# HKUDS/SSLRec

Measured on AMD Instinct MI355X. Metric: propagation_edges_per_sec, higher is better.
Workload: dtype f32

## Files before the change

include/sslrec_hip.h:

```cpp
#ifndef SSLREC_HIP_H
#define SSLREC_HIP_H

#include <stddef.h>
#include <stdint.h>

#ifdef __cplusplus
extern "C" {
#endif

#define SSLREC_ABI_VERSION 7
#define SSLREC_E_BADARG 1001

int sslrec_abi_version(void);

int sslrec_row_bits3(const int64_t *idx0, int64_t off0, const int64_t *idx1, int64_t off1, const int64_t *idx2, int64_t off2,
                     int32_t n, int32_t n_rows, uint32_t *bits, void *stream);

typedef struct sslrec_csr {
    int32_t n_rows, n_cols, nnz;
    int32_t d;
    int32_t n_elem;
    const int32_t *col;
    const float   *val;
    int32_t n_waves;
// ... 118 lines not shown
                             int32_t *w_len_out, void *stream);

typedef struct sslrec_plan sslrec_plan_t;
#define SSLREC_PLAN_AUTO 0
#define SSLREC_PLAN_SWEPT 1
#define SSLREC_PLAN_STREAMED 2
#define SSLREC_PLAN_BUNDLED 3
#define SSLREC_PLAN_NO_XCD_SPLIT 1
typedef struct sslrec_plan_info {
    int32_t n_rows, n_cols; int64_t nnz;
    int32_t kind, d, xcd_split;
    int32_t n_elem, n_blocks, n_slots, n_streams, n_rseg, n_long;
    int64_t xcd_col_pairs;
} sslrec_plan_info_t;
int sslrec_plan_build_coo(const int64_t *rows, const int64_t *cols, const float *vals, int64_t nnz, int32_t n_rows,
                          int32_t n_cols, sslrec_plan_t **out);
int sslrec_plan_build_csr(const int64_t *rowptr, const int32_t *col, const float *val, int32_t n_rows, int32_t n_cols,
                          sslrec_plan_t **out);
int sslrec_plan_set_option(sslrec_plan_t *p, const char *name, int64_t value);
int sslrec_plan_layout(sslrec_plan_t *p, int32_t d, int32_t kind, int32_t flags);
int sslrec_plan_info(const sslrec_plan_t *p, int32_t d, int32_t kind, sslrec_plan_info_t *info);
int sslrec_plan_host_array(const sslrec_plan_t *p, int32_t d, int32_t kind, const char *name, const void **ptr, int64_t *count,
                           int32_t *elem_bytes);
int sslrec_plan_upload(sslrec_plan_t *p, int32_t d, int32_t kind, void *stream);
const sslrec_swept_t *sslrec_plan_swept(const sslrec_plan_t *p, int32_t d);
const sslrec_csr_t *sslrec_plan_csr(const sslrec_plan_t *p, int32_t d);
const sslrec_bundled_t *sslrec_plan_bundled(const sslrec_plan_t *p, int32_t d);
const int32_t *sslrec_plan_edge_map(const sslrec_plan_t *p, int32_t d, int32_t kind);
int sslrec_plan_spmm_f32(const sslrec_plan_t *p, int32_t d, const float *X, float *Y, const sslrec_epilogue_t *epi,
                         void *stream);
void sslrec_plan_free(sslrec_plan_t *p);

int sslrec_debug_swept_trace(int enable, unsigned long long *host_out, int n_waves);

int sslrec_debug_stamp_next_launch(unsigned long long *record);
int sslrec_debug_wall_clock_khz(void);

size_t sslrec_bpr_ws_bytes(int32_t B);
size_t sslrec_bpr_bwd_ws_bytes(int32_t B, int32_t d);
int sslrec_bpr_fwd_f32(const float *Ta, const int64_t *ia, const float *Tp, const int64_t *ip,
                       const float *Tn, const int64_t *in, int32_t B, int32_t d, int32_t variant,
                       float divisor, float *ws, float *loss_out, void *stream);
int sslrec_bpr_fwd_total_f32(const float *Ta, const int64_t *ia, const float *Tp, const int64_t *ip,
                             const float *Tn, const int64_t *in, int32_t B, int32_t d, int32_t variant,
                             float divisor, const float *add_in, float *ws, float *loss_out2, void *stream);
int sslrec_bpr_bwd_f32(const float *Ta, const int64_t *ia, const float *Tp, const int64_t *ip,
                       const float *Tn, const int64_t *in, int32_t B, int32_t d, int32_t variant, float divisor,
                       const float *gscale_dev, float *dTa, float *dTp, float *dTn, void *ws, void *stream);
int sslrec_bpr_bwd_table_init(void *ws, int32_t B, int32_t d, void *stream);
int sslrec_bpr_bwd_kept_f32(const float *Ta, const int64_t *ia, const float *Tp, const int64_t *ip,
                            const float *Tn, const int64_t *in, int32_t B, int32_t d, int32_t variant, float divisor,
                            const float *gscale_dev, float *dTa, float *dTp, float *dTn, void *ws, float *zero_table,
                            size_t zero_elems, void *stream);

#define SSLREC_INFONCE_PREC_DEFAULT 0
#define SSLREC_INFONCE_PREC_X6 1
#define SSLREC_INFONCE_PREC_FP32 2
#define SSLREC_INFONCE_PREC_X36 3
#define SSLREC_INFONCE_PREC_X3 4
#define SSLREC_INFONCE_PREC_X63 5
#define SSLREC_INFONCE_PREC_X6A 6
#define SSLREC_INFONCE_PREC_H3 7
#define SSLREC_INFONCE_FWD_W (1 << 16)
size_t sslrec_infonce_ws_bytes(int32_t B, int32_t M, int32_t d);
int sslrec_infonce_fwd_f32(const float *T1, const int64_t *i1, const float *T2, const int64_t *i2,
                           int32_t B, const float *ALL, int32_t M, int32_t d, float temp,
                           int32_t variant, float *ws, float *loss_out, void *stream);
int sslrec_infonce_bwd_f32(const float *T1, const int64_t *i1, const float *T2, const int64_t *i2,
                           int32_t B, const float *ALL, int32_t M, int32_t d, float temp,
                           int32_t variant, float *ws, const float *gscale_dev,
                           float *dE1, float *dE2, float *dALL, void *stream);

int sslrec_infonce_bwd_scatter_f32(const float *T1, const int64_t *i1, const float *T2, const int64_t *i2,
                                   int32_t B, const float *ALL, int32_t M, int32_t d, float temp,
                                   int32_t variant, float *ws, const float *gscale_dev, float *dE,
                                   float *dT1, float *dT2, float *dALL, void *scatter_ws, void *stream);

int sslrec_infonce_shard_rowsum_f32(const float *T1, const int64_t *i1, const float *T2, const int64_t *i2,
                                    int32_t B, const float *ALL, int32_t M, int32_t d, float temp,
                                    int32_t variant, float *ws, float *z_part, void *stream);
int sslrec_infonce_shard_loss_f32(int32_t B, int32_t M, int32_t d, int32_t variant, float *ws,
                                  const float *z_total, float *loss_out, void *stream);
int sslrec_infonce_shard_bwd_f32(int32_t B, int32_t M, int32_t d, float temp, int32_t variant, float *ws,
                                 const float *gscale_dev, float *w_part, float *dALL, void *stream);
int sslrec_infonce_shard_finish_bwd_f32(int32_t B, int32_t M, int32_t d, float temp, int32_t variant,
                                        float *ws, const float *gscale_dev, const float *w_total,
                                        float *dE1, float *dE2, void *stream);

size_t sslrec_sumsq_ws_bytes(void);
int sslrec_sumsq_fwd_f32(const float *x, size_t n, float weight, float *ws, float *out, void *stream);
int sslrec_sumsq_bwd_f32(const float *x, size_t n, float weight, const float *gscale_dev, float *dx, void *stream);

int sslrec_weighted_sum4_f32(const float *t0, float w0, const float *t1, float w1, const float *t2, float w2, const float *t3, float w3,
                             float *out6, void *stream);
int sslrec_scalar_scale2_f32(const float *x, float a, float b, float *out2, void *stream);
int sslrec_add_tables_f32(const float *a, const float *b, const float *c, float *out, size_t n, void *stream);

int sslrec_adam_tick(float *state, double lr, double beta1, double beta2, void *stream);
int sslrec_adam_apply_f32(float *p, const float *g, float *m, float *v, size_t n, const float *state,
                          double beta1, double beta2, double eps, double weight_decay, void *stream);

size_t sslrec_rankq_ws_bytes(int32_t q, int32_t d);
int sslrec_rankq_reduce_f32(const float *M, int64_t stride_q, int64_t stride_n, const float *X, int32_t N, int32_t d,
                            int32_t q, float *ws, float *out, void *stream);
int sslrec_rankq_expand_f32(const float *M, int64_t stride_q, int64_t stride_n, const float *S, int32_t N, int32_t d,
                            int32_t q, float *Y, void *stream);
// ... 27 lines not shown
```

sslrec_amd/_lib.py:

```python
import ctypes as C
import os
import subprocess

_HERE = os.path.dirname(os.path.abspath(__file__))
CSRC = os.path.join(_HERE, 'csrc')
SO_PATH = os.environ.get('SSLREC_HIP_LIBRARY') or os.path.join(CSRC, 'libsslrec_hip.so')

E_BADARG = 1001
EXPECTED_ABI = 7


class CsrStruct(C.Structure):
    _fields_ = [
        ('n_rows', C.c_int32), ('n_cols', C.c_int32), ('nnz', C.c_int32), ('d', C.c_int32), ('n_elem', C.c_int32),
        ('col', C.c_void_p), ('val', C.c_void_p),
        ('n_waves', C.c_int32),
        ('w_start', C.c_void_p), ('w_len', C.c_void_p), ('r_ptr', C.c_void_p),
        ('n_rseg', C.c_int32),
        ('r_len', C.c_void_p), ('r_dst', C.c_void_p),
        ('n_long', C.c_int32),
        ('long_row', C.c_void_p), ('long_ptr', C.c_void_p),
        ('n_slots', C.c_int32),
    ]

# ... 55 lines not shown
    'sslrec_debug_stamp_next_launch': (C.c_int, [C.c_void_p]),
    'sslrec_debug_wall_clock_khz': (C.c_int, []),
    'sslrec_philox_row_sumsq': (C.c_int, [_P, C.c_uint32, _I, _I, _P, _P]),
    'sslrec_row_sumsq_f32': (C.c_int, [_P, _I, _I, _P, _P]),
    'sslrec_debug_gather_rows': (C.c_int, [_P, C.c_uint32, _I, _I, _I, _P, _P, _P]),
    'sslrec_debug_swept_trace': (C.c_int, [C.c_int, _P, C.c_int]),
    'sslrec_spmm_csr_f32': (C.c_int, [C.POINTER(CsrStruct), _P, _P, _P, _P, _P, _I, _P, C.POINTER(EpilogueStruct), _P, _P]),
    'sslrec_spmm_bundled_f32': (C.c_int, [C.POINTER(BundledStruct), _P, _P, _I, _P, C.POINTER(EpilogueStruct), _P, _P]),
    'sslrec_spmm_swept_f32': (C.c_int, [C.POINTER(SweptStruct), _P, _P, _P, _P, _I, _P, C.POINTER(EpilogueStruct), _P]),
    'sslrec_swept_deferred_sum_ok': (C.c_int, [C.POINTER(SweptStruct)]),
    'sslrec_spmm_swept_views_f32': (C.c_int, [C.POINTER(SweptStruct), _P, _I, C.POINTER(EpilogueViewsStruct), _P]),
    'sslrec_swept_compact': (C.c_int, [C.POINTER(SweptStruct), _P, _P, _F, _P, _P, _P, _P]),
    'sslrec_edge_drop_compact': (C.c_int, [C.POINTER(CsrStruct), _P, _P, _F, _P, _P, _P, _P, _P]),
    'sslrec_full_predict_f32': (C.c_int, [_P, _P, _I, _P, _I, _I, _P, _I, _P, _P]),
    'sslrec_eval_topk_ws_bytes': (C.c_size_t, [_I, _I, _I]),
    'sslrec_eval_topk_f32': (C.c_int, [_P, _P, _I, _P, _I, _I, _P, _P, _I, _P, _P, _P, _P]),
    'sslrec_sample_negs': (C.c_int, [_P, C.c_int64, _P, _P, _I, _P, C.c_uint32, _P, _P]),
    'sslrec_sample_negs_mt19937': (C.c_int, [_P, _P, _P, C.c_int64, _P, _P, _I, _I, _P, _P]),
    'sslrec_philox_advance': (C.c_int, [_P, _P]),
    'sslrec_philox_fill_f32': (C.c_int, [_P, C.c_uint32, _P, C.c_size_t, _P]),
    'sslrec_mt19937_uniform_f32': (C.c_int, [_P, _P, C.c_int64, _P]),
    'sslrec_mt19937_keep_mask': (C.c_int, [_P, C.c_float, _P, C.c_int64, _P]),
    'sslrec_mt19937_jump_poly': (C.c_int, [_P, _P, _P, _P]),
    'sslrec_mt19937_par_ws_bytes': (C.c_size_t, [C.c_int32, C.c_int32]),
    'sslrec_mt19937_uniform_par_f32': (C.c_int, [_P, _P, C.c_int32, C.c_int32, C.c_int64, _P, _P, C.c_int64, _P]),
    'sslrec_mt19937_keep_mask_par': (C.c_int, [_P, _P, C.c_int32, C.c_int32, C.c_int64, _P, C.c_float, _P, C.c_int64, _P]),
    'sslrec_swept_compact_philox': (C.c_int, [C.POINTER(SweptStruct), _P, _F, _P, C.c_uint32, _F, _P, _P, _P, _P]),
    'sslrec_edge_drop_compact_philox': (C.c_int, [C.POINTER(CsrStruct), _P, _F, _P, C.c_uint32, _F, _P, _P, _P, _P, _P]),
    'sslrec_bundled_drop_values': (C.c_int, [C.POINTER(BundledStruct), _P, _P, _F, _P, C.c_uint32, _F, _P, _P]),
    'sslrec_bundled_compact': (C.c_int, [C.POINTER(BundledStruct), _P, _P, _F, _P, _P, _P, _P, _P]),
    'sslrec_bundled_compact_philox': (C.c_int, [C.POINTER(BundledStruct), _P, _F, _P, C.c_uint32, _F, _P, _P, _P, _P, _P]),
    'sslrec_spmm_bundled_view_f32': (C.c_int, [C.POINTER(BundledStruct), _P, _P, _P, _P, _P, _I, _P, C.POINTER(EpilogueStruct), _P, _P]),
    'sslrec_plan_build_coo': (C.c_int, [_P, _P, _P, C.c_int64, _I, _I, C.POINTER(C.c_void_p)]),
    'sslrec_plan_build_csr': (C.c_int, [_P, _P, _P, _I, _I, C.POINTER(C.c_void_p)]),
    'sslrec_plan_set_option': (C.c_int, [_P, C.c_char_p, C.c_int64]),
    'sslrec_plan_layout': (C.c_int, [_P, _I, _I, _I]),
    'sslrec_plan_info': (C.c_int, [_P, _I, _I, C.POINTER(PlanInfoStruct)]),
    'sslrec_plan_host_array': (C.c_int, [_P, _I, _I, C.c_char_p, C.POINTER(C.c_void_p), C.POINTER(C.c_int64), C.POINTER(C.c_int32)]),
    'sslrec_plan_upload': (C.c_int, [_P, _I, _I, _P]),
    'sslrec_plan_swept': (C.c_void_p, [_P, _I]),
    'sslrec_plan_csr': (C.c_void_p, [_P, _I]),
    'sslrec_plan_bundled': (C.c_void_p, [_P, _I]),
    'sslrec_plan_edge_map': (C.c_void_p, [_P, _I, _I]),
    'sslrec_plan_spmm_f32': (C.c_int, [_P, _I, _P, _P, C.POINTER(EpilogueStruct), _P]),
    'sslrec_plan_free': (None, [_P]),
    'sslrec_bpr_ws_bytes': (C.c_size_t, [_I]),
    'sslrec_bpr_fwd_f32': (C.c_int, [_P, _P, _P, _P, _P, _P, _I, _I, _I, _F, _P, _P, _P]),
    'sslrec_bpr_fwd_total_f32': (C.c_int, [_P, _P, _P, _P, _P, _P, _I, _I, _I, _F, _P, _P, _P, _P]),
    'sslrec_bpr_bwd_ws_bytes': (C.c_size_t, [_I, _I]),
    'sslrec_scatter_ws_bytes': (C.c_size_t, [_I]),
    'sslrec_bpr_bwd_f32': (C.c_int, [_P, _P, _P, _P, _P, _P, _I, _I, _I, _F, _P, _P, _P, _P, _P, _P]),
    'sslrec_bpr_bwd_table_init': (C.c_int, [_P, _I, _I, _P]),
    'sslrec_bpr_bwd_kept_f32': (C.c_int, [_P, _P, _P, _P, _P, _P, _I, _I, _I, _F, _P, _P, _P, _P, _P, _P, C.c_size_t, _P]),
    'sslrec_infonce_ws_bytes': (C.c_size_t, [_I, _I, _I]),
    'sslrec_infonce_fwd_f32': (C.c_int, [_P, _P, _P, _P, _I, _P, _I, _I, _F, _I, _P, _P, _P]),
    'sslrec_infonce_bwd_f32': (C.c_int, [_P, _P, _P, _P, _I, _P, _I, _I, _F, _I, _P, _P, _P, _P, _P, _P]),
    'sslrec_infonce_bwd_scatter_f32': (C.c_int, [_P, _P, _P, _P, _I, _P, _I, _I, _F, _I, _P, _P, _P, _P, _P, _P, _P, _P]),
    'sslrec_infonce_shard_rowsum_f32': (C.c_int, [_P, _P, _P, _P, _I, _P, _I, _I, _F, _I, _P, _P, _P]),
    'sslrec_infonce_shard_loss_f32': (C.c_int, [_I, _I, _I, _I, _P, _P, _P, _P]),
    'sslrec_infonce_shard_bwd_f32': (C.c_int, [_I, _I, _I, _F, _I, _P, _P, _P, _P, _P]),
    'sslrec_infonce_shard_finish_bwd_f32': (C.c_int, [_I, _I, _I, _F, _I, _P, _P, _P, _P, _P, _P]),
    'sslrec_adam_tick': (C.c_int, [_P, C.c_double, C.c_double, C.c_double, _P]),
    'sslrec_adam_apply_f32': (C.c_int, [_P, _P, _P, _P, C.c_size_t, _P, C.c_double, C.c_double, C.c_double, C.c_double, _P]),
    'sslrec_rankq_ws_bytes': (C.c_size_t, [_I, _I]),
    'sslrec_rankq_reduce_f32': (C.c_int, [_P, C.c_int64, C.c_int64, _P, _I, _I, _I, _P, _P, _P]),
    'sslrec_rankq_expand_f32': (C.c_int, [_P, C.c_int64, C.c_int64, _P, _I, _I, _I, _P, _P]),
    'sslrec_scatter_add_rows_f32': (C.c_int, [_P, _P, _I, _I, _P, _P, _P]),
    'sslrec_sumsq_ws_bytes': (C.c_size_t, []),
    'sslrec_sumsq_fwd_f32': (C.c_int, [_P, C.c_size_t, _F, _P, _P, _P]),
    'sslrec_sumsq_bwd_f32': (C.c_int, [_P, C.c_size_t, _F, _P, _P, _P]),
    'sslrec_weighted_sum4_f32': (C.c_int, [_P, _F, _P, _F, _P, _F, _P, _F, _P, _P]),
    'sslrec_scalar_scale2_f32': (C.c_int, [_P, _F, _F, _P, _P]),
    'sslrec_add_tables_f32': (C.c_int, [_P, _P, _P, _P, C.c_size_t, _P]),
}

_lib = None


def build(force=False):
    if force and os.path.exists(SO_PATH):
        os.remove(SO_PATH)
    subprocess.run(['make', '-C', CSRC], check=True)
    return SO_PATH


def load():
    global _lib
    if _lib is not None:
        return _lib
    if not os.path.exists(SO_PATH):
        raise RuntimeError(
            'libsslrec_hip.so is not built (%s). Run `python __graft_entry__.py` or `make -C sslrec_amd/csrc`. '
            'sslrec_amd has no CPU / PyTorch fallback for its kernels by design.' % SO_PATH)
    lib = C.CDLL(SO_PATH)
    for name, (res, args) in SIGNATURES.items():
        fn = getattr(lib, name)
        fn.restype = res
        fn.argtypes = args
    got = lib.sslrec_abi_version()
    if got != EXPECTED_ABI:
        raise RuntimeError('%s implements ABI version %d, these bindings expect %d: rebuild the library '
                           '(`make -C sslrec_amd/csrc` or `python __graft_entry__.py`)' % (SO_PATH, got, EXPECTED_ABI))
    _lib = lib
    return lib


# ... 5 lines not shown
```

sslrec_amd/csrc/losses.hip:

```cpp
#include "common.h"
#include "det_scatter.h"
#include <stdlib.h>

typedef float f32x4 __attribute__((ext_vector_type(4)));

#define BPR_BLOCKS 256

__device__ __forceinline__ float bpr_term(float x, int variant) {
    if (variant == 0) {
        return (x > 20.f) ? x : log1pf(expf(x));
    }
    return -logf(1.f / (1.f + expf(x)));
}

__device__ __forceinline__ float bpr_dterm(float x, int variant) {
    if (variant == 0 && x > 20.f) return 1.f;
    return 1.f / (1.f + expf(-x));
}

__device__ __forceinline__ int64_t row_of(const int64_t *idx, int b) { return idx ? idx[b] : (int64_t)b; }

#if defined(__HIP_DEVICE_COMPILE__) && !defined(__gfx950__) && !defined(__gfx942__)
#error "finish_by_last_block relies on gfx942 / gfx950 atomics completing at the coherence point: use release / acquire on this target"
#endif
// ... 211 lines not shown
    float *G = (float *)ws;
    const DetTable tab = det_table(G + (size_t)3 * B * d);
    if (!kept_clean) {
        hipLaunchKernelGGL(det_clear_kernel, dim3(64), dim3(256), 0, st, tab);
        SSLREC_LAUNCH_CHECK();
    }
    hipLaunchKernelGGL(bpr_bwd_stage_kernel, dim3(blocks), dim3(256), 0, st, Ta, ia, Tp, ip, Tn, in, B, d, variant, divisor,
                       gscale_dev, dTa, dTp, dTn, G, tab, 0, reinterpret_cast<f32x4 *>(zero_table), zero_elems / 4);
    SSLREC_LAUNCH_CHECK();
    return det_reduce(tab, 3 * B, G, d, st, kept_clean ? 1 : 0);
}

extern "C" int sslrec_bpr_bwd_f32(const float *Ta, const int64_t *ia, const float *Tp, const int64_t *ip,
                                  const float *Tn, const int64_t *in, int32_t B, int32_t d, int32_t variant, float divisor,
                                  const float *gscale_dev, float *dTa, float *dTp, float *dTn, void *ws, void *stream) {
    return bpr_bwd_any(Ta, ia, Tp, ip, Tn, in, B, d, variant, divisor, gscale_dev, dTa, dTp, dTn, ws, stream, false);
}

extern "C" int sslrec_bpr_bwd_table_init(void *ws, int32_t B, int32_t d, void *stream) {
    if (!ws || B <= 0 || d <= 0 || 3 * (size_t)B > DET_MAX || d > 256) return SSLREC_E_BADARG;
    hipLaunchKernelGGL(det_clear_kernel, dim3(64), dim3(256), 0, (hipStream_t)stream, det_table((float *)ws + (size_t)3 * B * d));
    SSLREC_LAUNCH_CHECK();
    return 0;
}

extern "C" int sslrec_bpr_bwd_kept_f32(const float *Ta, const int64_t *ia, const float *Tp, const int64_t *ip,
                                       const float *Tn, const int64_t *in, int32_t B, int32_t d, int32_t variant, float divisor,
                                       const float *gscale_dev, float *dTa, float *dTp, float *dTn, void *ws, float *zero_table,
                                       size_t zero_elems, void *stream) {
    if (!ws || 3 * (size_t)B > DET_MAX || d > 256) return SSLREC_E_BADARG;
    return bpr_bwd_any(Ta, ia, Tp, ip, Tn, in, B, d, variant, divisor, gscale_dev, dTa, dTp, dTn, ws, stream, true, zero_table, zero_elems);
}

extern "C" int sslrec_scatter_add_rows_f32(const float *src, const int64_t *idx, int32_t B, int32_t d,
                                           float *dst, void *ws, void *stream) {
    if (!src || !idx || !dst || B < 0 || d <= 0) return SSLREC_E_BADARG;
    if (B == 0) return 0;
    hipStream_t st = (hipStream_t)stream;
    if (!ws || B > DET_MAX || d > 256) {
        int blocks = (B + 3) / 4;
        if (blocks > 2048) blocks = 2048;
        hipLaunchKernelGGL(scatter_add_rows_kernel, dim3(blocks), dim3(256), 0, st, src, idx, B, d, dst);
        SSLREC_LAUNCH_CHECK();
        return 0;
    }
    const DetTable tab = det_table(ws);
    hipLaunchKernelGGL(det_clear_kernel, dim3(64), dim3(256), 0, st, tab);
    SSLREC_LAUNCH_CHECK();
    hipLaunchKernelGGL(scatter_insert_kernel, dim3((B + 255) / 256), dim3(256), 0, st, idx, B, d, dst, tab);
    SSLREC_LAUNCH_CHECK();
    return det_reduce(tab, B, src, d, st);
}

#define SUMSQ_BLOCKS 1024

__global__ __launch_bounds__(256) void sumsq_kernel(const float *x, size_t n, float *ws, float weight, float *out, int one_launch) {
    __shared__ float wsum[4];
    const int lane = threadIdx.x & 63;
    float acc = 0.f;
    const size_t n4 = n / 4;
    const f32x4 *x4 = reinterpret_cast<const f32x4 *>(x);
    for (size_t i = (size_t)blockIdx.x * 256 + threadIdx.x; i < n4; i += (size_t)gridDim.x * 256) {
        const f32x4 v = x4[i];
        acc = fmaf(v[0], v[0], acc);
        acc = fmaf(v[1], v[1], acc);
        acc = fmaf(v[2], v[2], acc);
        acc = fmaf(v[3], v[3], acc);
    }
    if (blockIdx.x == 0 && threadIdx.x < (n & 3)) {
        const float v = x[n4 * 4 + threadIdx.x];
        acc = fmaf(v, v, acc);
    }
    acc = wave_sum(acc);
    if (lane == 0) wsum[threadIdx.x >> 6] = acc;
    __syncthreads();
    finish_by_last_block(ws, (wsum[0] + wsum[1]) + (wsum[2] + wsum[3]), gridDim.x, weight, 1.f, nullptr, out, one_launch);
}

__global__ __launch_bounds__(256) void scale2_kernel(const float *x, size_t n, const float *g, float weight, float *out) {
    const float s = 2.f * (g[0] * weight);
    const size_t n4 = n / 4;
    const f32x4 *x4 = reinterpret_cast<const f32x4 *>(x);
    f32x4 *o4 = reinterpret_cast<f32x4 *>(out);
    for (size_t i = (size_t)blockIdx.x * 256 + threadIdx.x; i < n4; i += (size_t)gridDim.x * 256) {
        f32x4 v = x4[i];
        v *= s;
        o4[i] = v;
    }
    if (blockIdx.x == 0 && threadIdx.x < (n & 3)) out[n4 * 4 + threadIdx.x] = s * x[n4 * 4 + threadIdx.x];
}

extern "C" size_t sslrec_sumsq_ws_bytes(void) { return (size_t)(FIN_PART0 + SUMSQ_BLOCKS) * sizeof(float); }

extern "C" int sslrec_sumsq_fwd_f32(const float *x, size_t n, float weight, float *ws, float *out, void *stream) {
    if (!x || !ws || !out || ((uintptr_t)x & 15)) return SSLREC_E_BADARG;
    hipStream_t st = (hipStream_t)stream;
    const int one = one_launch_reduce() ? 1 : 0;
    hipLaunchKernelGGL(sumsq_kernel, dim3(SUMSQ_BLOCKS), dim3(256), 0, st, x, n, ws, weight, out, one);
    SSLREC_LAUNCH_CHECK();
    if (!one) {
        hipLaunchKernelGGL(finish_partials_kernel, dim3(1), dim3(256), 0, st, ws, SUMSQ_BLOCKS, weight, 1.f, (const float *)nullptr, out);
        SSLREC_LAUNCH_CHECK();
    }
    return 0;
}

// ... 354 lines not shown
```

sslrec_amd/ops.py:

```python
import ctypes as C

import os

import torch

from . import _lib
from .graph import BundledLayout, DroppedView, PropGraph, RevaluedView, graph_of

PROFILE = None
PROFILE_EVERY = 1
_profile_tick = 0


def _profile_this_launch():
    global _profile_tick
    if PROFILE is None:
        return False
    _profile_tick += 1
    return PROFILE_EVERY <= 1 or _profile_tick % PROFILE_EVERY == 0


PROFILE_INFONCE = None

STAMPS = None
# ... 40 lines not shown
        if adj.scale != 1.0:
            return None
        graph = adj.graph
    elif isinstance(adj, PropGraph):
        graph = adj
    else:
        return None
    if graph.bwd is None:
        return None
    fact = graph.factorization()
    if fact is None or not fact[2]:
        return None
    if graph.fwd.swept(d) is None or graph.bwd.swept(d) is None:
        return None
    return fact[0]
MAX_SUM_IN = 3
DEFERRED_SUM = os.environ.get('SSLREC_DEFERRED_SUM', '0') == '1'
SPMM_NARROW_DIMS = (8, 16)
INFONCE_DIMS = (32, 64, 128)
EVAL_KMAX = 64
INFONCE_PRECISIONS = {None: 0, 'x6': 1, 'fp32': 2, 'x36': 3, 'x3': 4, 'x63': 5, 'x6a': 6, 'h3': 7}
INFONCE_FWD_W_BIT = 1 << 16
INFONCE_FWD_W = os.environ.get('SSLREC_INFONCE_FWD_W', '1') != '0'


def _variant_code(variant, precision):
    if precision not in INFONCE_PRECISIONS:
        raise ValueError('unknown InfoNCE precision %r (one of %s)' % (precision, sorted(k for k in INFONCE_PRECISIONS if k)))
    return int(variant) | (INFONCE_PRECISIONS[precision] << 8)


def _stream():
    return torch.cuda.current_stream().cuda_stream


_TICKET_WS = {}


def _ticket_ws(device, n_bytes, kind):
    dev = torch.device(device)
    key = (dev.index if dev.index is not None else torch.cuda.current_device(), kind)
    cur = torch.cuda.current_stream(dev)
    ent = _TICKET_WS.get(key)
    if ent is None or ent[0].numel() * 4 < n_bytes:
        ent = _TICKET_WS[key] = [torch.zeros(max(n_bytes // 4, 1), dtype=torch.float32, device=dev), cur]
    elif ent[1] != cur:
        if not torch.cuda.is_current_stream_capturing():
            cur.wait_stream(ent[1])
        ent[1] = cur
    return ent[0]


import collections
import threading

_KEPT_WS = collections.OrderedDict()
_KEPT_WS_MAX = 8
_KEPT_WS_LOCK = threading.Lock()
SSLREC_KEPT_SCATTER = os.environ.get('SSLREC_KEPT_SCATTER', '1') != '0'


def _bpr_bwd_ws(device, B, d):
    lib = _lib.load()
    n = lib.sslrec_bpr_bwd_ws_bytes(B, d) // 4 + 1
    if not SSLREC_KEPT_SCATTER or 3 * B > 16384 or d > 256 or B <= 0:
        return torch.empty(n, dtype=torch.float32, device=device), False
    dev = torch.device(device)
    key = (dev.index if dev.index is not None else torch.cuda.current_device(), int(B), int(d))
    cur = torch.cuda.current_stream(dev)
    with _KEPT_WS_LOCK:
        ent = _KEPT_WS.get(key)
        if ent is None:
            ws = torch.empty(n, dtype=torch.float32, device=dev)
            _lib.check(lib.sslrec_bpr_bwd_table_init(ws.data_ptr(), int(B), int(d), _stream()), 'sslrec_bpr_bwd_table_init')
            ent = _KEPT_WS[key] = [ws, cur]
            while len(_KEPT_WS) > _KEPT_WS_MAX and not torch.cuda.is_current_stream_capturing():
                _k, old_ent = _KEPT_WS.popitem(last=False)
                if old_ent[1] is not None:
                    old_ent[0].record_stream(old_ent[1])
        else:
            _KEPT_WS.move_to_end(key)
            if ent[1] != cur:
                if not torch.cuda.is_current_stream_capturing():
                    cur.wait_stream(ent[1])
                ent[1] = cur
    return ent[0], True


def _check_kept(rc, what, device, B, d):
    if rc != 0:
        dev = torch.device(device)
        with _KEPT_WS_LOCK:
            _KEPT_WS.pop((dev.index if dev.index is not None else torch.cuda.current_device(), int(B), int(d)), None)
    _lib.check(rc, what)


def _need_gpu(*tensors):
    for t in tensors:
        if t is not None and not t.is_cuda:
            raise RuntimeError('sslrec_amd kernels run on a HIP device only (got a %s tensor); there is no CPU '
                               'fallback by design' % t.device)


def _f32c(t):
    if t.dtype != torch.float32:
        raise TypeError('fp32 tensors expected, got %s' % t.dtype)
    return t if t.is_contiguous() else t.contiguous()


def _idx(t):
    if t is None:
        return None
    if t.dtype != torch.int64:
        t = t.long()
    return t if t.is_contiguous() else t.contiguous()


def _ptr(t):
    return 0 if t is None else t.data_ptr()


def spmm_raw(adj, x, which='fwd', y=None, noise=None, eps=0.0, acc_in=None, acc_out=None, want_y=True, chained=False,
             noise_sumsq=None, noise_geom=None, axpy=None, x_row_bits=None, sum_in=None, row_scale=None, scale_flags=0):
    view = adj if isinstance(adj, (DroppedView, RevaluedView)) else None
    graph = adj.graph if view is not None else adj
    plan = getattr(graph, which)
    _need_gpu(x)
    x = _f32c(x)
    n, d = x.shape
    if n != plan.n_cols:
        raise ValueError('operand has %d rows, matrix has %d columns' % (n, plan.n_cols))
    if d not in SPMM_DIMS and d not in SPMM_NARROW_DIMS:
        raise ValueError('embedding size %d not supported by the raw HIP SpMM launcher (supported: %s and %s); the ops.spmm / '
                         'ops.propagate_sum wrappers zero-pad other sizes' % (d, SPMM_NARROW_DIMS, SPMM_DIMS))
    if want_y and y is None:
        y = torch.empty((plan.n_rows, d), dtype=torch.float32, device=x.device)
    epi = None
    keep_alive = []
    if noise is not None or acc_out is not None or x_row_bits is not None or scale_flags:
# ... 428 lines not shown
        return out.reshape(())

    @staticmethod
    def backward(ctx, g):
        ta, tp, tn, ia, ip, in_ = ctx.saved_tensors
        ia = ia if ctx.has_idx[0] else None
        ip = ip if ctx.has_idx[1] else None
        in_ = in_ if ctx.has_idx[2] else None
        B, d, variant, shared_pn, divisor = ctx.meta
        g = g.reshape(1).to(torch.float32).contiguous()
        dta = torch.zeros_like(ta) if ia is not None else torch.empty_like(ta)
        if shared_pn:
            dtp = torch.zeros_like(tp)
            dtn = dtp
        else:
            dtp = torch.zeros_like(tp) if ip is not None else torch.empty_like(tp)
            dtn = torch.zeros_like(tn) if in_ is not None else torch.empty_like(tn)
        lib = _lib.load()
        ws, kept = _bpr_bwd_ws(ta.device, B, d)
        args = (ta.data_ptr(), _ptr(ia), tp.data_ptr(), _ptr(ip), tn.data_ptr(), _ptr(in_), B, d,
                variant, divisor, g.data_ptr(), dta.data_ptr(), dtp.data_ptr(), dtn.data_ptr(), ws.data_ptr())
        rc = lib.sslrec_bpr_bwd_kept_f32(*args, None, 0, _stream()) if kept else lib.sslrec_bpr_bwd_f32(*args, _stream())
        _check_kept(rc, 'sslrec_bpr_bwd_f32', ta.device, B, d)
        return dta, dtp, (None if shared_pn else dtn), None, None, None, None, None, None


def bpr_loss_and_grads(anc, pos, neg, variant=0, divisor=1.0):
    _need_gpu(anc, pos, neg)
    anc, pos, neg = _f32c(anc.detach()), _f32c(pos.detach()), _f32c(neg.detach())
    B, d = anc.shape
    lib = _lib.load()
    dev = anc.device
    ws = _ticket_ws(dev, lib.sslrec_bpr_ws_bytes(B), 'bpr')
    out = torch.empty(1, dtype=torch.float32, device=dev)
    rc = lib.sslrec_bpr_fwd_f32(anc.data_ptr(), None, pos.data_ptr(), None, neg.data_ptr(), None, B, d, int(variant),
                                float(divisor), ws.data_ptr(), out.data_ptr(), _stream())
    _lib.check(rc, 'sslrec_bpr_fwd_f32')
    one = torch.ones(1, dtype=torch.float32, device=dev)
    da, dp, dn = torch.empty_like(anc), torch.empty_like(pos), torch.empty_like(neg)
    ws2 = torch.empty(lib.sslrec_bpr_bwd_ws_bytes(B, d) // 4 + 1, dtype=torch.float32, device=dev)
    rc = lib.sslrec_bpr_bwd_f32(anc.data_ptr(), None, pos.data_ptr(), None, neg.data_ptr(), None, B, d, int(variant),
                                float(divisor), one.data_ptr(), da.data_ptr(), dp.data_ptr(), dn.data_ptr(), ws2.data_ptr(), _stream())
    _lib.check(rc, 'sslrec_bpr_bwd_f32')
    return out, da, dp, dn


def bpr_loss(anc, pos, neg, variant=0, divisor=1.0):
    return _BprFn.apply(anc, pos, neg, None, None, None, int(variant), False, float(divisor))


class _BprStackedFn(torch.autograd.Function):

    @staticmethod
    def forward(ctx, table, n_user, ancs, poss, negs, variant, divisor, add):
        _need_gpu(table)
        table = _f32c(table)
        ia, ip, in_ = _idx(ancs), _idx(poss), _idx(negs)
        B, d = int(ia.numel()), table.shape[1]
        lib = _lib.load()
        ws = _ticket_ws(table.device, lib.sslrec_bpr_ws_bytes(B), 'bpr')
        p = table.data_ptr()
        pi = p + int(n_user) * d * 4
        ctx.save_for_backward(table, ia, ip, in_)
        ctx.meta = (B, d, variant, int(n_user), float(divisor))
        ctx.two = add is not None
        ctx.set_materialize_grads(False)
        if add is None:
            out = torch.empty(1, dtype=torch.float32, device=table.device)
            rc = lib.sslrec_bpr_fwd_f32(p, ia.data_ptr(), pi, ip.data_ptr(), pi, in_.data_ptr(), B, d, variant, float(divisor),
                                        ws.data_ptr(), out.data_ptr(), _stream())
            _lib.check(rc, 'sslrec_bpr_fwd_f32')
            return out.reshape(())
        _need_gpu(add)
        addc = add.detach().reshape(1).to(torch.float32).contiguous()
        out = torch.empty(2, dtype=torch.float32, device=table.device)
        rc = lib.sslrec_bpr_fwd_total_f32(p, ia.data_ptr(), pi, ip.data_ptr(), pi, in_.data_ptr(), B, d, variant, float(divisor),
                                          addc.data_ptr(), ws.data_ptr(), out.data_ptr(), _stream())
        _lib.check(rc, 'sslrec_bpr_fwd_total_f32')
        return out[1].reshape(()), out[0].reshape(())

    @staticmethod
    def backward(ctx, *grads):
        table, ia, ip, in_ = ctx.saved_tensors
        B, d, variant, n_user, divisor = ctx.meta
        if ctx.two:
            g_total, g_bpr = grads
            g_add = g_total
            g = g_total if g_bpr is None else (g_bpr if g_total is None else g_total + g_bpr)
        else:
            g, g_add = grads[0], None
        if g is None:
            return None, None, None, None, None, None, None, g_add
        g = g.reshape(1).to(torch.float32).contiguous()
        lib = _lib.load()
        ws, kept = _bpr_bwd_ws(table.device, B, d)
        fused_zero = kept and B > 0 and table.numel() % 4 == 0
        grad = torch.empty_like(table) if fused_zero else torch.zeros_like(table)
        p, q = table.data_ptr(), grad.data_ptr()
        pi, qi = p + n_user * d * 4, q + n_user * d * 4
        args = (p, ia.data_ptr(), pi, ip.data_ptr(), pi, in_.data_ptr(), B, d, variant, divisor, g.data_ptr(), q, qi, qi, ws.data_ptr())
        if kept:
            rc = lib.sslrec_bpr_bwd_kept_f32(*args, q if fused_zero else None, grad.numel() if fused_zero else 0, _stream())
        else:
            rc = lib.sslrec_bpr_bwd_f32(*args, _stream())
        _check_kept(rc, 'sslrec_bpr_bwd_f32', table.device, B, d)
        if SPARSE_GRAD:
            _tag_row_bits(grad, RowBits.from_indices(table.shape[0], ia, 0, ip, n_user, in_, n_user))
        return grad, None, None, None, None, None, None, g_add


def bpr_loss_stacked(table, n_user, ancs, poss, negs, variant=0, divisor=1.0, add=None):
    return _BprStackedFn.apply(table, int(n_user), ancs, poss, negs, int(variant), float(divisor), add)


def bpr_loss_gathered(user_table, item_table, ancs, poss, negs, variant=0, divisor=1.0):
    return _BprFn.apply(user_table, item_table, item_table, ancs, poss, negs, int(variant), True, float(divisor))


def _infonce_event():
    if PROFILE_INFONCE is None:
        return None
    ev = torch.cuda.Event(enable_timing=True)
    ev.record()
    return ev


def _infonce_record(ev0, kind, B, M, d, variant):
    if ev0 is not None and PROFILE_INFONCE is not None:
        ev1 = torch.cuda.Event(enable_timing=True)
        ev1.record()
        PROFILE_INFONCE.append((ev0, ev1, kind, B, M, d, variant))


def infonce_issued_flops(kind, B, M, d, variant):
    code = (variant >> 8) & 0xFF
    v1 = (variant & 0xFF) != 0
    if code == 0:
        v1_default = 'x6' if (os.environ.get('SSLREC_INFONCE_V1_DEFAULT') or 'h3')[0] == 'x' else 'h3'
        code = INFONCE_PRECISIONS.get(os.environ.get('SSLREC_INFONCE_PRECISION') or (v1_default if v1 else 'h3'), 1)
    if v1 and code not in (2, 7):
        code = 1
    fwd_w = bool(variant & INFONCE_FWD_W_BIT) and not (code == 2 and d == 128)
    sc, wa, da = {1: (6, 6, 6), 2: (1, 1, 1), 3: (3, 6, 6), 4: (3, 3, 3), 5: (6, 3, 3), 6: (6, 6, 3), 7: (3, 3, 3)}[code]
    unit = 2.0 * B * M * d
    pre = 1 if (v1 and code == 7 and (kind == 'fwd')) else 0
    if kind == 'fwd':
        f = sc + (wa if fwd_w else 0) + pre
    else:
        f = sc + da + (0 if fwd_w else sc + wa)
    return f * unit, ('fp32' if code == 2 else ('fp16' if code == 7 else 'bf16'))


class _InfoNceFn(torch.autograd.Function):
    @staticmethod
    def forward(ctx, t1, t2, all_, i1, i2, temp, variant, t2_is_all, will_differentiate=True):
        _need_gpu(t1, t2, all_)
        t1, t2, all_ = _f32c(t1), _f32c(t2), _f32c(all_)
        i1, i2 = _idx(i1), _idx(i2)
        B = int(i1.numel()) if i1 is not None else t1.shape[0]
        M, d = all_.shape
        if d not in INFONCE_DIMS:
            raise ValueError('embedding size %d not supported by the HIP InfoNCE (supported: %s)' % (d, INFONCE_DIMS))
        lib = _lib.load()
        if INFONCE_FWD_W and will_differentiate and any(ctx.needs_input_grad[:3]):
            variant |= INFONCE_FWD_W_BIT
# ... 519 lines not shown
```

Measured before the change: 56.44 billion.

## Fuse BPR forward with deterministic scatter-table build and backward zero-fill

Adds a stacked BPR forward kernel that computes dot products for several samples per wave. When armed for training, it also inserts gathered rows into the deterministic scatter table, sets touched-row bits, and stashes the per-sample derivative. The matching backward kernel writes each touched gradient row deterministically and zeroes only untouched rows, so the separate table-build pass and full zero-fill go away. The price is more complex workspace arming and lifetime tracking through weakrefs, plus atomics in the forward pass.

```diff
diff --git a/include/sslrec_hip.h b/include/sslrec_hip.h
--- a/include/sslrec_hip.h
+++ b/include/sslrec_hip.h
@@ -194,6 +194,13 @@
                             const float *Tn, const int64_t *in, int32_t B, int32_t d, int32_t variant, float divisor,
                             const float *gscale_dev, float *dTa, float *dTp, float *dTn, void *ws, float *zero_table,
                             size_t zero_elems, void *stream);
+size_t sslrec_bpr_stacked_zero_bytes(int32_t B, int32_t d, int32_t n_rows);
+int sslrec_bpr_fwd_stacked_f32(const float *table, int32_t n_rows, int32_t n_user, const int64_t *ia, const int64_t *ip,
+                               const int64_t *in, int32_t B, int32_t d, int32_t variant, float divisor, const float *add_in,
+                               float *ws, void *kept_ws, float *loss_out, void *stream);
+int sslrec_bpr_bwd_stacked_f32(const float *table, int32_t n_rows, int32_t n_user, const int64_t *ia, const int64_t *ip,
+                               const int64_t *in, int32_t B, int32_t d, int32_t variant, float divisor, const float *gscale_dev,
+                               float *grad, void *kept_ws, void *stream);
 
 #define SSLREC_INFONCE_PREC_DEFAULT 0
 #define SSLREC_INFONCE_PREC_X6 1
diff --git a/sslrec_amd/_lib.py b/sslrec_amd/_lib.py
--- a/sslrec_amd/_lib.py
+++ b/sslrec_amd/_lib.py
@@ -131,6 +131,9 @@
     'sslrec_bpr_bwd_f32': (C.c_int, [_P, _P, _P, _P, _P, _P, _I, _I, _I, _F, _P, _P, _P, _P, _P, _P]),
     'sslrec_bpr_bwd_table_init': (C.c_int, [_P, _I, _I, _P]),
     'sslrec_bpr_bwd_kept_f32': (C.c_int, [_P, _P, _P, _P, _P, _P, _I, _I, _I, _F, _P, _P, _P, _P, _P, _P, C.c_size_t, _P]),
+    'sslrec_bpr_stacked_zero_bytes': (C.c_size_t, [_I, _I, _I]),
+    'sslrec_bpr_fwd_stacked_f32': (C.c_int, [_P, _I, _I, _P, _P, _P, _I, _I, _I, _F, _P, _P, _P, _P, _P]),
+    'sslrec_bpr_bwd_stacked_f32': (C.c_int, [_P, _I, _I, _P, _P, _P, _I, _I, _I, _F, _P, _P, _P, _P]),
     'sslrec_infonce_ws_bytes': (C.c_size_t, [_I, _I, _I]),
     'sslrec_infonce_fwd_f32': (C.c_int, [_P, _P, _P, _P, _I, _P, _I, _I, _F, _I, _P, _P, _P]),
     'sslrec_infonce_bwd_f32': (C.c_int, [_P, _P, _P, _P, _I, _P, _I, _I, _F, _I, _P, _P, _P, _P, _P, _P]),
diff --git a/sslrec_amd/csrc/losses.hip b/sslrec_amd/csrc/losses.hip
--- a/sslrec_amd/csrc/losses.hip
+++ b/sslrec_amd/csrc/losses.hip
@@ -287,6 +287,225 @@
     return det_reduce(tab, B, src, d, st);
 }
 
+#define BPR_FWD_U 4
+
+struct BprFused {
+    DetTable tab;
+    uint32_t *bits;
+    float *stash;
+};
+
+static size_t bpr_fused_bits_bytes(int B, int d, int n_rows) {
+    if (B <= 0 || d <= 0 || n_rows <= 0 || 3 * (size_t)B > DET_MAX || d > 256 || (d & 3)) return 0;
+    const size_t bits = (((size_t)(n_rows + 31) / 32) * 4 + 15) & ~(size_t)15;
+    return bits + (size_t)B * 4 <= (size_t)3 * B * d * 4 ? bits : 0;
+}
+
+static BprFused bpr_fused(void *ws, int B, int d, int n_rows) {
+    BprFused f;
+    f.tab = det_table((float *)ws + (size_t)3 * B * d);
+    f.bits = (uint32_t *)ws;
+    f.stash = (float *)((char *)ws + bpr_fused_bits_bytes(B, d, n_rows));
+    return f;
+}
+
+template <bool INS>
+__global__ __launch_bounds__(256) void bpr_fwd_stacked_kernel(const float *__restrict__ T, int n_user, const int64_t *__restrict__ ia,
+                                                              const int64_t *__restrict__ ip, const int64_t *__restrict__ in, int B, int d,
+                                                              int variant, float *ws, float divisor, const float *add_in, float *out,
+                                                              int one_launch, BprFused fz) {
+    __shared__ float wsum[4];
+    const int lane = threadIdx.x & 63;
+    const int w = wave_in_block();
+    const int nw = gridDim.x * 4;
+    const float *Ti = T + (size_t)n_user * d;
+    float local = 0.f;
+    for (int b0 = blockIdx.x * 4 + w; b0 < B; b0 += BPR_FWD_U * nw) {
+        int64_t ra[BPR_FWD_U], rp[BPR_FWD_U], rn[BPR_FWD_U];
+#pragma unroll
+        for (int u = 0; u < BPR_FWD_U; ++u) {
+            const int b = b0 + u * nw;
+            const bool ok = b < B;
+            ra[u] = ok ? ia[b] : 0;
+            rp[u] = ok ? ip[b] : 0;
+            rn[u] = ok ? in[b] : 0;
+        }
+        const int iu = lane / 3, role = lane - 3 * (lane / 3);
+        float dp[BPR_FWD_U], dn[BPR_FWD_U];
+#pragma unroll
+        for (int u = 0; u < BPR_FWD_U; ++u) dp[u] = dn[u] = 0.f;
+        for (int k = lane; k < d; k += 64) {
+            float av[BPR_FWD_U], pv[BPR_FWD_U], nv[BPR_FWD_U];
+#pragma unroll
+            for (int u = 0; u < BPR_FWD_U; ++u) {
+                const bool ok = b0 + u * nw < B;
+                av[u] = ok ? T[ra[u] * d + k] : 0.f;
+                pv[u] = ok ? Ti[rp[u] * d + k] : 0.f;
+                nv[u] = ok ? Ti[rn[u] * d + k] : 0.f;
+            }
+            if constexpr (INS) {
+                if (k == lane) {
+                    int64_t r = 0;
+#pragma unroll
+                    for (int v = 0; v < BPR_FWD_U; ++v)
+                        if (iu == v) r = role == 0 ? ra[v] : (role == 1 ? rp[v] : rn[v]);
+                    const int b = b0 + iu * nw;
+                    if (iu < BPR_FWD_U && b < B) {
+                        const int64_t row = role == 0 ? r : n_user + r;
+                        det_insert(fz.tab, T + row * d, 3 * b + role);
+                        atomicOr(fz.bits + (row >> 5), 1u << (row & 31));
+                    }
+                }
+            }
+#pragma unroll
+            for (int u = 0; u < BPR_FWD_U; ++u) {
+                dp[u] = fmaf(av[u], pv[u], dp[u]);
+                dn[u] = fmaf(av[u], nv[u], dn[u]);
+            }
+        }
+#pragma unroll
+        for (int u = 0; u < BPR_FWD_U; ++u) {
+            dp[u] = wave_sum(dp[u]);
+            dn[u] = wave_sum(dn[u]);
+        }
+#pragma unroll
+        for (int u = 0; u < BPR_FWD_U; ++u)
+            if (b0 + u * nw < B) local += bpr_term(dn[u] - dp[u], variant);
+        if constexpr (INS) {
+            float x = 0.f;
+#pragma unroll
+            for (int v = 0; v < BPR_FWD_U; ++v)
+                if (iu == v) x = dn[v] - dp[v];
+            const int b = b0 + iu * nw;
+            if (iu < BPR_FWD_U && role == 0 && b < B) fz.stash[b] = bpr_dterm(x, variant);
+        }
+    }
+    if (lane == 0) wsum[w] = local;
+    __syncthreads();
+    finish_by_last_block(ws, (wsum[0] + wsum[1]) + (wsum[2] + wsum[3]), gridDim.x, 1.f, divisor, add_in, out, one_launch);
+}
+
+__device__ __forceinline__ float bpr_contrib(const float *T, const float *Ti, const int64_t *ia, const int64_t *ip, const int64_t *in,
+                                             int d, float g, const float *stash, int e, int k) {
+    const int b = e / 3, role = e - 3 * b;
+    const float s = g * stash[b];
+    if (role == 0) {
+        const float pv = Ti[ip[b] * d + k], nv = Ti[in[b] * d + k];
+        return s * (nv - pv);
+    }
+    const float av = T[ia[b] * d + k];
+    return role == 1 ? -s * av : s * av;
+}
+
+__global__ __launch_bounds__(256) void bpr_bwd_stacked_kernel(const float *__restrict__ T, int n_user, const int64_t *__restrict__ ia,
+                                                              const int64_t *__restrict__ ip, const int64_t *__restrict__ in, int B, int d,
+                                                              float divisor, const float *gscale, float *grad, int n_rows, BprFused fz) {
+#pragma clang fp contract(off)
+    const int lane = threadIdx.x & 63;
+    const int K = 3 * B, n_words = (n_rows + 31) / 32, dv = d / 4;
+    const float *Ti = T + (size_t)n_user * d;
+    const float g = gscale[0] / divisor;
+    const DetTable &t = fz.tab;
+#define BPR_RELEASE_SLOT() if (lane == 0) { t.key[slot] = 0ull; t.cnt[slot] = 0; t.first[slot] = 0x7fffffff; }
+    for (int task = blockIdx.x * 4 + wave_in_block(); task < K + n_words; task += gridDim.x * 4) {
+        if (task >= K) {
+            const int wd = task - K, r0 = wd * 32;
+            const uint32_t word = fz.bits[wd];
+            const int nr = min(32, n_rows - r0);
+            f32x4 *g4 = reinterpret_cast<f32x4 *>(grad + (size_t)r0 * d);
+            for (int j = lane; j < nr * dv; j += 64)
+                if (!((word >> (j / dv)) & 1u)) g4[j] = f32x4{0.f, 0.f, 0.f, 0.f};
+            if (lane == 0 && word) fz.bits[wd] = 0u;
+            continue;
+        }
+        const int e = task;
+        const int slot = t.slot_of[e];
+        const int c = t.cnt[slot];
+        const int b = e / 3, role = e - 3 * b;
+        float *row = grad + (size_t)(role == 0 ? ia[b] : n_user + (role == 1 ? ip[b] : in[b])) * d;
+        if (c == 1) {
+            for (int k = lane; k < d; k += 64) row[k] = 0.f + bpr_contrib(T, Ti, ia, ip, in, d, g, fz.stash, e, k);
+            BPR_RELEASE_SLOT()
+            continue;
+        }
+        if (t.first[slot] != e) continue;
+        if (c <= DET_LIST) {
+            int ids[DET_LIST];
+#pragma unroll
+            for (int i = 0; i < DET_LIST; ++i) ids[i] = i < c ? t.list[(size_t)slot * DET_LIST + i] : 0x7fffffff;
+#pragma unroll
+            for (int i = 1; i < DET_LIST; ++i)
+#pragma unroll
+                for (int j = i; j > 0; --j)
+                    if (ids[j] < ids[j - 1]) { const int x = ids[j]; ids[j] = ids[j - 1]; ids[j - 1] = x; }
+            for (int k = lane; k < d; k += 64) {
+                float acc = 0.f;
+#pragma unroll
+                for (int i = 0; i < DET_LIST; ++i)
+                    if (i < c) acc += bpr_contrib(T, Ti, ia, ip, in, d, g, fz.stash, ids[i], k);
+                row[k] = 0.f + acc;
+            }
+        } else {
+            float acc[4] = {0.f, 0.f, 0.f, 0.f};
+            for (int j0 = 0; j0 < K; j0 += 64) {
+                const int j = j0 + lane;
+                unsigned long long m = __ballot(j < K && t.slot_of[j] == slot);
+                while (m) {
+                    const int id = j0 + __ffsll((long long)m) - 1;
+                    m &= m - 1;
+#pragma unroll
+                    for (int q = 0; q < 4; ++q)
+                        if (lane + 64 * q < d) acc[q] += bpr_contrib(T, Ti, ia, ip, in, d, g, fz.stash, id, lane + 64 * q);
+                }
+            }
+#pragma unroll
+            for (int q = 0; q < 4; ++q)
+                if (lane + 64 * q < d) row[lane + 64 * q] = 0.f + acc[q];
+        }
+        BPR_RELEASE_SLOT()
+    }
+#undef BPR_RELEASE_SLOT
+}
+
+extern "C" size_t sslrec_bpr_stacked_zero_bytes(int32_t B, int32_t d, int32_t n_rows) { return bpr_fused_bits_bytes(B, d, n_rows); }
+
+extern "C" int sslrec_bpr_fwd_stacked_f32(const float *table, int32_t n_rows, int32_t n_user, const int64_t *ia, const int64_t *ip,
+                                          const int64_t *in, int32_t B, int32_t d, int32_t variant, float divisor, const float *add_in,
+                                          float *ws, void *kept_ws, float *loss_out, void *stream) {
+    if (!table || !ia || !ip || !in || !ws || !loss_out || B < 0 || d <= 0 || n_user < 0 || n_user > n_rows ||
+        (variant != 0 && variant != 1) || !(divisor != 0.f))
+        return SSLREC_E_BADARG;
+    if (kept_ws && !bpr_fused_bits_bytes(B, d, n_rows)) return SSLREC_E_BADARG;
+    hipStream_t st = (hipStream_t)stream;
+    const int one = one_launch_reduce() ? 1 : 0;
+    if (kept_ws)
+        hipLaunchKernelGGL(bpr_fwd_stacked_kernel<true>, dim3(BPR_BLOCKS), dim3(256), 0, st, table, n_user, ia, ip, in, B, d, variant, ws,
+                           divisor, add_in, loss_out, one, bpr_fused(kept_ws, B, d, n_rows));
+    else
+        hipLaunchKernelGGL(bpr_fwd_stacked_kernel<false>, dim3(BPR_BLOCKS), dim3(256), 0, st, table, n_user, ia, ip, in, B, d, variant, ws,
+                           divisor, add_in, loss_out, one, BprFused{});
+    SSLREC_LAUNCH_CHECK();
+    if (!one) {
+        hipLaunchKernelGGL(finish_partials_kernel, dim3(1), dim3(256), 0, st, ws, BPR_BLOCKS, 1.f, divisor, add_in, loss_out);
+        SSLREC_LAUNCH_CHECK();
+    }
+    return 0;
+}
+
+extern "C" int sslrec_bpr_bwd_stacked_f32(const float *table, int32_t n_rows, int32_t n_user, const int64_t *ia, const int64_t *ip,
+                                          const int64_t *in, int32_t B, int32_t d, int32_t variant, float divisor,
+                                          const float *gscale_dev, float *grad, void *kept_ws, void *stream) {
+    if (!table || !ia || !ip || !in || !gscale_dev || !grad || !kept_ws || n_user < 0 || n_user > n_rows || (variant != 0 && variant != 1) ||
+        ((uintptr_t)grad & 15) || !(divisor != 0.f) || !bpr_fused_bits_bytes(B, d, n_rows))
+        return SSLREC_E_BADARG;
+    const long tasks = 3L * B + (n_rows + 31) / 32;
+    const int blocks = (int)((tasks + 3) / 4 < 8192 ? (tasks + 3) / 4 : 8192);
+    hipLaunchKernelGGL(bpr_bwd_stacked_kernel, dim3(blocks), dim3(256), 0, (hipStream_t)stream, table, n_user, ia, ip, in, B, d, divisor,
+                       gscale_dev, grad, n_rows, bpr_fused(kept_ws, B, d, n_rows));
+    SSLREC_LAUNCH_CHECK();
+    return 0;
+}
+
 #define SUMSQ_BLOCKS 1024
 
 __global__ __launch_bounds__(256) void sumsq_kernel(const float *x, size_t n, float *ws, float weight, float *out, int one_launch) {
diff --git a/sslrec_amd/ops.py b/sslrec_amd/ops.py
--- a/sslrec_amd/ops.py
+++ b/sslrec_amd/ops.py
@@ -116,6 +116,7 @@
 
 
 import collections
+import weakref
 import threading
 
 _KEPT_WS = collections.OrderedDict()
@@ -124,7 +125,7 @@
 SSLREC_KEPT_SCATTER = os.environ.get('SSLREC_KEPT_SCATTER', '1') != '0'
 
 
-def _bpr_bwd_ws(device, B, d):
+def _bpr_bwd_ws(device, B, d, arming=False):
     lib = _lib.load()
     n = lib.sslrec_bpr_bwd_ws_bytes(B, d) // 4 + 1
     if not SSLREC_KEPT_SCATTER or 3 * B > 16384 or d > 256 or B <= 0:
@@ -148,7 +149,66 @@
                 if not torch.cuda.is_current_stream_capturing():
                     cur.wait_stream(ent[1])
                 ent[1] = cur
+        if not arming:
+            st = _kept_arm_state(key, ent[0], B, d)
+            if st is None:
+                return torch.empty(n, dtype=torch.float32, device=device), False
+            st[2] = 0
     return ent[0], True
+
+
+FUSED_BPR = os.environ.get('SSLREC_FUSED_BPR', '1') != '0'
+_KEPT_ARM = {}
+
+
+class _FusedHold:
+    """held by the autograd node whose forward armed a kept workspace (sslrec_bpr_fwd_stacked_f32); the workspace is clean again once
+    that node's backward ran.  A node freed without its backward leaves the table armed: the next user re-initialises it."""
+
+
+def _kept_arm_state(key, ws, B, d):
+    st = _KEPT_ARM.get(key)
+    if st is None or st[0] is not ws:
+        st = _KEPT_ARM[key] = [ws, None, 0]
+    if st[1] is not None:
+        if st[1]() is not None:
+            return None
+        st[1], st[2] = None, 0
+        _lib.check(_lib.load().sslrec_bpr_bwd_table_init(ws.data_ptr(), int(B), int(d), _stream()), 'sslrec_bpr_bwd_table_init')
+    return st
+
+
+def _bpr_fused_acquire(device, B, d, n_rows):
+    if not (FUSED_BPR and SSLREC_KEPT_SCATTER):
+        return None, None
+    need = _lib.load().sslrec_bpr_stacked_zero_bytes(int(B), int(d), int(n_rows))
+    if need == 0:
+        return None, None
+    ws, kept = _bpr_bwd_ws(device, B, d, arming=True)
+    if not kept:
+        return None, None
+    dev = torch.device(device)
+    key = (dev.index if dev.index is not None else torch.cuda.current_device(), int(B), int(d))
+    with _KEPT_WS_LOCK:
+        st = _kept_arm_state(key, ws, B, d)
+        if st is None:
+            return None, None
+        if st[2] < need:
+            ws[:need // 4].zero_()
+            st[2] = need
+        hold = _FusedHold()
+        st[1] = weakref.ref(hold)
+    return st, hold
+
+
+def _bpr_fused_release(st, key, ok):
+    with _KEPT_WS_LOCK:
+        st[1] = None
+        if not ok:
+            ent = _KEPT_WS.get(key)
+            if ent is not None and ent[0] is st[0]:
+                del _KEPT_WS[key]
+            _KEPT_ARM.pop(key, None)
 
 
 def _check_kept(rc, what, device, B, d):
@@ -683,7 +743,7 @@
 class _BprStackedFn(torch.autograd.Function):
 
     @staticmethod
-    def forward(ctx, table, n_user, ancs, poss, negs, variant, divisor, add):
+    def forward(ctx, table, n_user, ancs, poss, negs, variant, divisor, add, arm=False):
         _need_gpu(table)
         table = _f32c(table)
         ia, ip, in_ = _idx(ancs), _idx(poss), _idx(negs)
@@ -696,6 +756,23 @@
         ctx.meta = (B, d, variant, int(n_user), float(divisor))
         ctx.two = add is not None
         ctx.set_materialize_grads(False)
+        ctx.fused = None
+        if FUSED_BPR and B > 0 and table.shape[0] < 2 ** 31:
+            st, hold = _bpr_fused_acquire(table.device, B, d, table.shape[0]) if arm else (None, None)
+            _need_gpu(add)
+            addc = None if add is None else add.detach().reshape(1).to(torch.float32).contiguous()
+            out = torch.empty(1 if add is None else 2, dtype=torch.float32, device=table.device)
+            rc = lib.sslrec_bpr_fwd_stacked_f32(p, table.shape[0], int(n_user), ia.data_ptr(), ip.data_ptr(), in_.data_ptr(), B, d, variant,
+                                                float(divisor), _ptr(addc), ws.data_ptr(), None if st is None else st[0].data_ptr(),
+                                                out.data_ptr(), _stream())
+            if st is not None:
+                key = (table.device.index if table.device.index is not None else torch.cuda.current_device(), B, d)
+                if rc != 0:
+                    _bpr_fused_release(st, key, False)
+                else:
+                    ctx.fused = (st, hold, key)
+            _lib.check(rc, 'sslrec_bpr_fwd_stacked_f32')
+            return out.reshape(()) if add is None else (out[1].reshape(()), out[0].reshape(()))
         if add is None:
             out = torch.empty(1, dtype=torch.float32, device=table.device)
             rc = lib.sslrec_bpr_fwd_f32(p, ia.data_ptr(), pi, ip.data_ptr(), pi, in_.data_ptr(), B, d, variant, float(divisor),
@@ -721,9 +798,21 @@
         else:
             g, g_add = grads[0], None
         if g is None:
-            return None, None, None, None, None, None, None, g_add
+            return None, None, None, None, None, None, None, g_add, None
         g = g.reshape(1).to(torch.float32).contiguous()
         lib = _lib.load()
+        fused, ctx.fused = ctx.fused, None
+        if fused is not None and fused[0][1] is not None and fused[0][1]() is fused[1]:
+            st, _hold, key = fused
+            _bpr_bwd_ws(table.device, B, d, arming=True)
+            grad = torch.empty_like(table)
+            rc = lib.sslrec_bpr_bwd_stacked_f32(table.data_ptr(), table.shape[0], n_user, ia.data_ptr(), ip.data_ptr(), in_.data_ptr(), B, d,
+                                                variant, divisor, g.data_ptr(), grad.data_ptr(), st[0].data_ptr(), _stream())
+            _bpr_fused_release(st, key, rc == 0)
+            _lib.check(rc, 'sslrec_bpr_bwd_stacked_f32')
+            if SPARSE_GRAD:
+                _tag_row_bits(grad, RowBits.from_indices(table.shape[0], ia, 0, ip, n_user, in_, n_user))
+            return grad, None, None, None, None, None, None, g_add, None
         ws, kept = _bpr_bwd_ws(table.device, B, d)
         fused_zero = kept and B > 0 and table.numel() % 4 == 0
         grad = torch.empty_like(table) if fused_zero else torch.zeros_like(table)
@@ -737,11 +826,12 @@
         _check_kept(rc, 'sslrec_bpr_bwd_f32', table.device, B, d)
         if SPARSE_GRAD:
             _tag_row_bits(grad, RowBits.from_indices(table.shape[0], ia, 0, ip, n_user, in_, n_user))
-        return grad, None, None, None, None, None, None, g_add
+        return grad, None, None, None, None, None, None, g_add, None
 
 
 def bpr_loss_stacked(table, n_user, ancs, poss, negs, variant=0, divisor=1.0, add=None):
-    return _BprStackedFn.apply(table, int(n_user), ancs, poss, negs, int(variant), float(divisor), add)
+    arm = torch.is_grad_enabled() and table.requires_grad
+    return _BprStackedFn.apply(table, int(n_user), ancs, poss, negs, int(variant), float(divisor), add, arm)
 
 
 def bpr_loss_gathered(user_table, item_table, ancs, poss, negs, variant=0, divisor=1.0):
```

After: 56.97 billion, median of 6. About the same (+0.9%).
